# dscripka/openWakeWord

Hardware: AMD Instinct MI355X
Metric: real-time audio frames/sec (80 ms frame, 3 wakewords), whole job; real-time streams = value/12.5 (higher is better)
Workload: dtype f32 as 3xf16 split MFMA, fp32 accumulate; 1 GPU; 131072 concurrent 16 kHz streams per GPU x 3 heads (alexa,hey_mycroft,hey_jarvis), 80 ms frames, BASELINE configs[3] per-GPU shard; streams_per_gpu=131072, frame_samples=1280, collective=none, gather=none, rccl_ranks=0, pcm_distribution=Gaussian, RMS 3000, pcm=resident in HBM, kernels=mfma_rr_f16x3, graph=False, vad=off, weights=synthetic seed 1234, step_blocks=1

## Files before the change

### openwakeword_amd/csrc/owwhip.hip

```cpp
#include <hip/hip_runtime.h>

#include <algorithm>
#include <cmath>
#include <cstdio>
#include <cstdlib>
#include <cstring>
#include <ctime>
#include <exception>
#include <mutex>
#include <new>
#include <unordered_map>
#include <dlfcn.h>
#include <string>
#include <vector>

#include "owwhip.h"
#include "owwhip_pack.h"
#include "owwhip_kernels.h"
#include "owwhip_rr.h"
#include "owwhip_hx.h"
#include "owwhip_vad.h"
#include "owwhip_fused.h"
#include "owwhip_state.h"
#include "owwhip_events.h"
// ... 164 lines not shown
        oww_event* h_rec = nullptr; int* h_count = nullptr;
    };
    int evt_cap = 0, evt_rows = 0;
    float* d_evt_thr = nullptr; float evt_bank_thr = 0.5f;
    int* d_evblock = nullptr; int evt_blocks = 0;
    EventBuf evt_sync, evt_slot[2];
    const EventBuf* evt_cur = nullptr;

    hipStream_t up_stream = nullptr, down_stream = nullptr;
    uint64_t n_submit = 0, n_collect = 0;
    float* d_featinit = nullptr;
    float* d_dbg = nullptr;
    long long* d_prof = nullptr;
    int prof_block = -1;
    uint32_t *d_nfeat = nullptr, *d_npred = nullptr;
    float* d_vadring = nullptr; uint32_t* d_nvad = nullptr; float* d_vadin = nullptr; float vad_threshold = 0.f;
    bool vad = false;
    const float *d_vad_hann = nullptr, *d_vad_encw = nullptr, *d_vad_encb = nullptr, *d_vad_lstmw = nullptr, *d_vad_lstmb = nullptr, *d_vad_wd = nullptr;
    float vad_bd = 0.f, vad_gain = 50.f;
    float *d_vadx = nullptr, *d_vadhc = nullptr, *d_vadlast = nullptr;
    int16_t *d_tail = nullptr, *d_pcm = nullptr;
    int16_t* d_long = nullptr; size_t long_cap = 0;
    float* d_callmax = nullptr;
    int* h_range = nullptr;
    int* d_range = nullptr;
    void* d_rs = nullptr; size_t rs_bytes = 0;
    std::vector<float> rs_taps;
    uint8_t* d_on = nullptr;
    int* d_lists = nullptr; int* h_lists[2] = {nullptr, nullptr}; hipEvent_t lists_ev[2] = {nullptr, nullptr}; size_t lists_cap = 0; unsigned lists_turn = 0;
    int k_last = 1;
    float hx_absmax[20] = {};
    std::vector<int16_t> cal_user;
    int small_wgs = kSmallLaunchWgs, small_wgs_heads = kSmallLaunchWgs;
    float hx_selftest_err = 0.f, hx_selftest_ref = 0.f, hx_selftest_score_err = 0.f;
    bool fuse = false;
    float *d_verw = nullptr, *d_verb = nullptr, *d_verthr = nullptr; int* d_verT = nullptr;
    int ver_stride = 0, n_verifiers = 0;
    std::vector<int> ver_T;
    bool post_in_heads = false;
    float* d_save = nullptr; size_t save_floats = 0;
    int* d_ids = nullptr;
    int ids_cap = 0;
    int *d_patience = nullptr;
    float* d_threshold = nullptr;
    int debounce_frames = 0;
    void* comm = nullptr; int comm_rank = 0, comm_world = 1;
    bool timing = false;
    std::vector<EventRec> ev;
    size_t ev_used = 0;
    double t_ms[OWW_N_KERNEL_CLASSES] = {};
    int64_t t_n[OWW_N_KERNEL_CLASSES] = {};
    bool want_graph = false;
    hipGraph_t graph = nullptr;
    hipGraphExec_t graph_exec = nullptr;
    struct BankHead {
        bool live = false;
        int T = 0, hidden = 0, has_ln = 0, ht = 4, patience = 0;
        float threshold = NAN;
        float* d_img = nullptr;
        size_t w1_bytes = 0;
        owh::BankHeadDev dev{};
    };
    int bank_K = 0, bank_cap = 0;
    std::vector<BankHead> bank;
    std::vector<int> bank_sub;
    int* d_bank_sub = nullptr; int* d_bank_idx = nullptr;
// ... 102 lines not shown
            p.w[i] = h->d_conv[first_layer + i]; p.scale[i] = h->d_scale[first_layer + i];
            p.shift[i] = h->d_shift[first_layer + i]; p.dbg_off[i] = dbg_off[first_layer + i];
        }
        p.dbg = dbg ? h->d_dbg : nullptr; p.dbg_stride = DBG_FLOATS;
        p.prof = h->d_prof ? h->d_prof + (first_layer / 4) * 256 : nullptr;
        p.prof_block = h->prof_block;
    };
    {
        StageParams p{}; fill(p, h->d_xA, h->d_xB, 3, 2, 3);
        Timed t(h, 2);
        hipLaunchKernelGGL((stage_kernel<CfgB, MFMA, false>), dim3((n_active + CfgB::B - 1) / CfgB::B), dim3(CfgB::NT), CfgB::LDS_BYTES, st, p);
    }
    {
        StageParams p{}; fill(p, h->d_xB, h->d_xC, 7, 4, 5);
        Timed t(h, 3);
        hipLaunchKernelGGL((stage_kernel<CfgC, MFMA, false>), dim3((n_active + CfgC::B - 1) / CfgC::B), dim3(CfgC::NT), CfgC::LDS_BYTES, st, p);
    }
    {
        StageParams p{}; fill(p, h->d_xC, h->d_xD, 11, 6, 7);
        Timed t(h, 4);
        hipLaunchKernelGGL((stage_kernel<CfgD, MFMA, false>), dim3((n_active + CfgD::B - 1) / CfgD::B), dim3(CfgD::NT), CfgD::LDS_BYTES, st, p);
    }
    {
        StageParams p{}; fill(p, h->d_xD, nullptr, 15, 8, 9);
        p.hist19 = h->d_state[10]; p.w19 = h->d_conv[19]; p.feat = h->d_feat; p.emb = h->d_emb; p.nfeat = h->d_nfeat; p.TR = h->TR;
        p.dbg_off[4] = dbg_off[19];
        Timed t(h, 5);
        hipLaunchKernelGGL((stage_kernel<CfgE, MFMA, true>), dim3((n_active + CfgE::B - 1) / CfgE::B), dim3(CfgE::NT), CfgE::LDS_BYTES, st, p);
    }
    HIPCHK(hipGetLastError());
    return 0;
}

template <class CR, class CH, int WG, bool LAST, bool DBG, bool HX>
void launch_rstage(oww_ctx* h, const owr::RStageParams& p, int cls) {
    hipStream_t st = h->stream;
    Timed t(h, cls);
    const int nwg = (p.n_groups + WG - 1) / WG;
    if (HX && !DBG && nwg <= h->small_wgs) hipLaunchKernelGGL((owh::hstage_kernel<CH, LAST, false, WG, 3>), dim3(nwg), dim3(64 * WG), 0, st, p);
    else if (HX) hipLaunchKernelGGL((owh::hstage_kernel<CH, LAST, DBG, WG>), dim3(nwg), dim3(64 * WG), 0, st, p);
    else hipLaunchKernelGGL((owr::rstage_kernel<CR, LAST, DBG>), dim3((p.n_groups + 3) / 4), dim3(256), 0, st, p);
}

template <bool DBG, bool HX>
int run_cnn_rr(oww_ctx* h, const StepArgs& a, int n_active, int mel_stride, int mel_off) {
    using namespace owr;
    hipStream_t st = h->stream;
    int off = 0, dbg_off[20];
    for (int l = 0; l < 20; ++l) { dbg_off[l] = off; off += kLayerOut[l][0] * kLayerOut[l][1] * kLayerOut[l][2]; }
    {
        RAParams p{};
        p.mel = a.mel ? a.mel : h->d_mel; p.mel_stride = mel_stride; p.mel_off = mel_off;
        p.hist_mel = h->d_state[0]; p.hist2 = h->d_state[1];
        p.w0 = h->d_conv[0]; p.w1 = h->d_conv[1]; p.w2 = h->d_conv[2];
        for (int i = 0; i < 3; ++i) { p.scale[i] = h->d_scale[i]; p.shift[i] = h->d_shift[i]; p.dbg_off[i] = dbg_off[i]; }
        p.xout = h->d_xA; p.n_streams = n_active; p.S = h->Spad;
        p.dbg = DBG ? h->d_dbg : nullptr; p.dbg_stride = DBG_FLOATS;
        for (int i = 0; i < 3; ++i) { p.clampv[i] = -0.4f * ldexpf(1.f, h->hx_e[i]); p.dbg_mul[i] = ldexpf(1.f, -h->hx_e[i]); }
        p.xmul = ldexpf(1.f, h->hx_xexp[0]);
        p.range_flag = HX ? h->d_range : nullptr;
        p.stream_on = a.on;
        const int grid = std::min((n_active + 3) / 4, 768);
        Timed t(h, 1);
        if (HX && a.fused_pcm) {
            owf::MelAParams q{};
            q.a = p; q.a.mel = nullptr; q.a.n_streams = h->S;
            q.pcm = a.fused_pcm; q.tail = h->d_tail; q.nfeat = h->d_nfeat; q.hann = h->d_hann; q.mel_start = h->d_mstart; q.mel_taps = h->d_taps; q.mel_off = h->d_meloff; q.mel_dst = h->d_meldst;
            q.mel_out = h->cfg.debug_layers ? h->d_mel : nullptr;
            const int per_cu = std::max(1, std::min(12 / owf::FA_WG, 163840 / owf::FA_LDS_BYTES));
            const int g2 = std::max(1, std::min((q.a.n_streams + owf::FA_WG - 1) / owf::FA_WG, 256 * per_cu));
            hipLaunchKernelGGL(owf::hmelA_kernel<DBG>, dim3(g2), dim3(64 * owf::FA_WG), owf::FA_LDS_BYTES, st, q);
        }
        else if (HX) hipLaunchKernelGGL(owh::hstageA_kernel<DBG>, dim3(std::min((n_active + 3) / 4, 256 * OWH_WPS_A)), dim3(256), 0, st, p);
        else hipLaunchKernelGGL(rstageA_kernel<DBG>, dim3(grid), dim3(256), 0, st, p);
    }
    auto fill = [&](const float* xin, float* xout, int first_layer, int sb, int sd, int spt) {
        RStageParams p{};
        p.xin = xin; p.xout = xout; p.hist_b = h->d_state[sb]; p.hist_d = h->d_state[sd];
        for (int i = 0; i < 4; ++i) {
            p.w[i] = h->d_conv[first_layer + i]; p.scale[i] = h->d_scale[first_layer + i];
            p.shift[i] = h->d_shift[first_layer + i]; p.dbg_off[i] = dbg_off[first_layer + i];
            p.clampv[i] = -0.4f * ldexpf(1.f, h->hx_e[first_layer + i]); p.dbg_mul[i] = ldexpf(1.f, -h->hx_e[first_layer + i]);
        }
        p.dbg_mul[4] = ldexpf(1.f, -h->hx_e[19]);
        p.xmul = ldexpf(1.f, h->hx_xexp[first_layer / 4 + 1]);
        p.emb_mul = ldexpf(1.f, -h->hx_e[19]);
        p.n_groups = (n_active + spt - 1) / spt; p.S = h->Spad;
        p.dbg = DBG ? h->d_dbg : nullptr; p.dbg_stride = DBG_FLOATS;
        p.range_flag = HX ? h->d_range : nullptr;
        p.stream_on = a.on;
        if (HX && a.lists) {
            const int k = spt == 1 ? 0 : spt == 2 ? 1 : spt == 4 ? 2 : 3;
            p.glist = a.gl[k]; p.n_groups = a.gn[k];
        }
        return p;
    };
    launch_rstage<RB, owh::HB, OWH_WG_B, false, DBG, HX>(h, fill(h->d_xA, h->d_xB, 3, 2, 3, RB::SPT), 2);
    launch_rstage<RC, owh::HC, OWH_WG_C, false, DBG, HX>(h, fill(h->d_xB, h->d_xC, 7, 4, 5, RC::SPT), 3);
    launch_rstage<RD, owh::HD, OWH_WG_D, false, DBG, HX>(h, fill(h->d_xC, h->d_xD, 11, 6, 7, RD::SPT), 4);
    RStageParams pe = fill(h->d_xD, nullptr, 15, 8, 9, RE::SPT);
    pe.hist19 = h->d_state[10]; pe.w19 = h->d_conv[19]; pe.feat = h->d_feat; pe.emb = h->d_emb; pe.nfeat = h->d_nfeat; pe.TR = h->TR;
    pe.dbg_off[4] = dbg_off[19];
    launch_rstage<RE, owh::HE, OWH_WG_E, true, DBG, HX>(h, pe, 5);
    HIPCHK(hipGetLastError());
    return 0;
}

int run_cnn(oww_ctx* h, const StepArgs& a, int n_active, int mel_stride, int mel_off) {
    n_active = std::min(h->Spad, (n_active + 7) / 8 * 8);
    if (h->hx) return a.dbg ? run_cnn_rr<true, true>(h, a, n_active, mel_stride, mel_off) : run_cnn_rr<false, true>(h, a, n_active, mel_stride, mel_off);
    if (h->rr) return a.dbg ? run_cnn_rr<true, false>(h, a, n_active, mel_stride, mel_off) : run_cnn_rr<false, false>(h, a, n_active, mel_stride, mel_off);
    return h->mfma ? run_cnn_t<true>(h, a, n_active, mel_stride, mel_off) : run_cnn_t<false>(h, a, n_active, mel_stride, mel_off);
}

int heads_lds_bytes(int NH) { return (HD_SB * 100 + 2 * HD_SB * (NH + 4) + HD_SB * HD_MAXNETS) * 4; }

void launch_generic_heads(oww_ctx* h, const HeadParams& p, int n_active, int nb, int ne, hipStream_t st) {
    const int hs = (std::max(h->generic_hmax, 1) + 3) & ~3;
    const bool big = h->generic_hmax <= 128 && (h->generic_spw == 16 || (h->generic_spw == 0 && n_active >= GH_BIG_STREAMS));
    if (big) hipLaunchKernelGGL((heads_generic_kernel<16, 2, 2>), dim3((n_active + 31) / 32), dim3(128), gh_lds_bytes(16, 2, hs), st, p, nb, ne, hs);
    else hipLaunchKernelGGL((heads_generic_kernel<4, 4>), dim3((n_active + 15) / 16), dim3(256), gh_lds_bytes(4, 4, hs), st, p, nb, ne, hs);
}

int run_heads(oww_ctx* h, const StepArgs& a, int n_active, bool accumulate_max, const float* ext, int only_head, float* raw_out, int force_generic) {
    hipStream_t st = h->stream;
    Timed t(h, 6);
    HeadParams base{};
    base.feat = ext ? ext : h->d_feat; base.ext = ext ? 1 : 0; base.TR = h->TR; base.nfeat = h->d_nfeat;
    base.raw = raw_out; base.NL = h->NL; base.S = n_active; base.accumulate_max = accumulate_max ? 1 : 0;
    base.stream_on = ext ? nullptr : a.on;
    const bool fast_ok = h->mfma && !force_generic;
    if (fast_ok) {
        for (auto& g : h->groups) {
            if (only_head >= 0) {
                bool has = false;
                for (int ni : g.nets) has |= h->nets[ni].head == only_head;
// ... 881 lines not shown
        const size_t G = (SP + 15) / 16;
        if (int rc = dalloc(h->stream, &h->d_vadx, G * 4 * 1024)) return rc;
        if (int rc = dalloc(h->stream, &h->d_vadhc, G * 4096)) return rc;
        if (int rc = dalloc(h->stream, &h->d_vadlast, SP)) return rc;
    }
    if (int rc = dalloc(h->stream, &h->d_tail, SP * 480)) return rc;
    if (int rc = dalloc(h->stream, &h->d_pcm, (size_t)h->S * OWW_CHUNK * h->kmax)) return rc;
    if (int rc = dalloc(h->stream, &h->d_patience, (size_t)std::max(h->NL, 1))) return rc;
    if (int rc = dalloc(h->stream, &h->d_threshold, (size_t)std::max(h->NL, 1))) return rc;
    {
        std::vector<float> nanv(std::max(h->NL, 1), NAN);
        HIPCHK(copy_async(h->d_threshold, nanv.data(), nanv.size() * sizeof(float), hipMemcpyHostToDevice, h->stream));
    }
    if (h->cfg.debug_layers) if (int rc = dalloc(h->stream, &h->d_dbg, SP * DBG_FLOATS)) return rc;
    if (const char* e = getenv("OWW_PROF_BLOCK")) { h->prof_block = atoi(e); if (int rc = dalloc(h->stream, &h->d_prof, (size_t)4 * 256)) return rc; }
    return 0;
}

int set_kernel_lds(oww_ctx* h) {
    int rc = 0;
    auto lds = [&rc](auto kernel, int bytes) { if (!rc) rc = set_lds(kernel, bytes); };
    for (const auto& g : h->groups) if (g.ht == 4) lds(heads64_kernel, heads_lds_bytes(g.NH));
    if (!h->rnn_nets.empty()) lds(heads_rnn_kernel<RNN_SPW>, (int)rnn_lds_bytes(RNN_TMAX));
    if (h->vad) lds(owv::vad_front_kernel, owv::V_LDS_BYTES);
    lds(owf::hmelA_kernel<false>, owf::FA_LDS_BYTES); lds(owf::hmelA_kernel<true>, owf::FA_LDS_BYTES);
    lds(stageA_kernel<true>, CfgA::LDS_BYTES); lds(stageA_kernel<false>, CfgA::LDS_BYTES);
    lds(stage_kernel<CfgB, true, false>, CfgB::LDS_BYTES); lds(stage_kernel<CfgB, false, false>, CfgB::LDS_BYTES);
    lds(stage_kernel<CfgC, true, false>, CfgC::LDS_BYTES); lds(stage_kernel<CfgC, false, false>, CfgC::LDS_BYTES);
    lds(stage_kernel<CfgD, true, false>, CfgD::LDS_BYTES); lds(stage_kernel<CfgD, false, false>, CfgD::LDS_BYTES);
    lds(stage_kernel<CfgE, true, true>, CfgE::LDS_BYTES); lds(stage_kernel<CfgE, false, true>, CfgE::LDS_BYTES);
    return rc;
}

int derive_reset_state(oww_ctx* h, const HxCalib& cal, CommitClock& clk) {
    const size_t SP = h->Spad;
    const int warm = std::min<int>(32, (int)SP);
    hipLaunchKernelGGL(fill_kernel, dim3((warm * 256 + 255) / 256), dim3(256), 0, h->stream, h->d_mel, (size_t)warm * 256, 1.0f);
    const StepArgs args{};
    for (int it = 0; it < 12; ++it)
        if (int rc = run_cnn(h, args, warm, 256, 0)) return rc;
    for (int a = 0; a < N_STATE; ++a)
        HIPCHK(copy_async(h->d_tmpl[a], h->d_state[a], (size_t)h->state_len[a] * (h->rr ? kStateSpgRr[a] : 1) * sizeof(float),
                              hipMemcpyDeviceToDevice, h->stream));
    HIPCHK(hipMemsetAsync(h->d_mel, 0, SP * 8 * h->kmax * 32 * sizeof(float), h->stream));
    HIPCHK(hipMemsetAsync(h->d_emb, 0, SP * 96 * sizeof(float), h->stream));
    if (int rc = do_reset(h, nullptr, (int)SP, nullptr)) return rc;
    HIPCHK(hipStreamSynchronize(h->stream));
    clk.lap("warm-up + reset");
    if (int rc = range_check(h, "oww_commit")) return rc;
    if (h->hx && !getenv("OWW_NO_COMMIT_SELFTEST")) {
        if (int rc = selftest_hx(h, cal)) return rc;
        HIPCHK(hipMemsetAsync(h->d_mel, 0, SP * 8 * h->kmax * 32 * sizeof(float), h->stream));
        HIPCHK(hipMemsetAsync(h->d_emb, 0, SP * 96 * sizeof(float), h->stream));
        HIPCHK(hipMemsetAsync(h->d_raw, 0, SP * std::max(h->NL, 1) * sizeof(float), h->stream));
        if (int rc = do_reset(h, nullptr, (int)SP, nullptr)) return rc;
        HIPCHK(hipStreamSynchronize(h->stream));
        clk.lap("self-test replay + reset");
    }
    return 0;
}

int alloc_bank(oww_ctx* h) {
    const size_t SK = (size_t)h->S * h->bank_K;
    if (int rc = dalloc(h->stream, &h->d_bank_sub, SK, false)) return rc;
    if (int rc = dalloc(h->stream, &h->d_bank_idx, SK)) return rc;
    if (int rc = dalloc(h->stream, &h->d_bank_raw, SK)) return rc;
// ... 330 lines not shown
    if (int rc = build_nets(*h, h->NL, h->TR, h->generic_hmax)) return rc;
    if (h->evt_rows > h->TR)
        return fail(OWW_EINVAL, "oww_events_configure: feature_rows = %d exceeds the handle's feature ring (%d rows)", h->evt_rows, h->TR);
    CommitClock clk(h->hx ? "f16-split" : "family");
    HxCalib cal;
    if (h->hx) {
        if (int rc = calibrate_hx(h, cal)) return rc;
        h->probe_emb = cal.ref_emb; h->probe_nb = cal.nb;
        clk.lap("calibration (total)");
        if (getenv("OWW_DEBUG_CALIB"))
            for (int l = 0; l < 20; ++l) fprintf(stderr, "calib layer %2d: max|a| %-12.5g e_in %4d e_out %4d\n", l, h->hx_absmax[l], h->hx_ein[l], h->hx_e[l]);
    }
    HostBuf hb;
    WeightOff off;
    HeadGroups hg;
    h->no_wide_heads = getenv("OWW_NO_WIDE_HEADS") != nullptr;
    if (int rc = pack_mel_tables(*h, hb, off)) return rc;
    if (int rc = pack_cnn(*h, hb, off)) return rc;
    pack_net_arrays(*h, hb, off);
    if (int rc = pack_head_groups(*h, hg, hb, off)) return rc;
    h->groups.clear();
    for (const HeadGroup& g : hg.groups) h->groups.push_back(FastGroup{g});
    h->generic_nets = hg.generic_nets; h->rnn_nets = hg.rnn_nets;
    h->vad = !h->vad_blob.empty();
    if (int rc = pack_vad(*h, hb, off, h->vad_gain, h->vad_bd)) return rc;
    clk.lap("weight packing (host)");
    if (int rc = bind_weights(h, hb, off)) return rc;
    if (int rc = alloc_range_flag(h)) return rc;
    clk.lap("weight upload");
    if (int rc = alloc_state(h)) return rc;
    h->fuse = h->hx && !getenv("OWW_NO_FUSE");
    if (const char* e = getenv("OWW_SMALL_WGS")) h->small_wgs = atoi(e);
    if (const char* e = getenv("OWW_SMALL_WGS_HEADS")) h->small_wgs_heads = atoi(e);
    if (const char* e = getenv("OWW_GENERIC_SPW")) { const int v = atoi(e); h->generic_spw = v == 4 || v == 16 ? v : 0; }
    h->post_in_heads = h->fuse && h->groups.size() == 1 && h->groups[0].ht == 4 && h->generic_nets.empty() && h->rnn_nets.empty() && h->NL > 0;
    if (int rc = set_kernel_lds(h)) return rc;
    clk.lap("state allocation");
    if (int rc = derive_reset_state(h, cal, clk)) return rc;
    if (h->bank_K > 0) if (int rc = alloc_bank(h)) return rc;
    if (h->vpool_cap > 0) if (int rc = alloc_verifiers(h)) return rc;
    if (events_on(h)) if (int rc = alloc_events(h)) return rc;
    h->committed = true;
    return OWW_OK;
    OWW_GUARD_END
}

int oww_reset(oww_ctx* h, const int32_t* stream_ids, int32_t n, const float* init_features) {
    OWW_GUARD_BEGIN
    if (!h || !h->committed) return fail(OWW_ESTATE, "oww_reset: handle not committed");
    HIPCHK(hipSetDevice(h->cfg.device));
    const float* d_init = nullptr;
    if (init_features) {
        HIPCHK(copy_async(h->d_featinit, init_features, (size_t)h->TR * 96 * sizeof(float), hipMemcpyHostToDevice, h->stream));
        d_init = h->d_featinit;
    }
    if (!stream_ids) {
        if (int rc = do_reset(h, nullptr, h->Spad, d_init)) return rc;
    } else {
        if (n < 1) return OWW_OK;
        for (int i = 0; i < n; ++i)
            if (stream_ids[i] < 0 || stream_ids[i] >= h->S) return fail(OWW_EINVAL, "oww_reset: stream id %d out of range", stream_ids[i]);
        if (n > h->ids_cap) {
            if (h->d_ids) (void)dev_free(h->d_ids);
            h->d_ids = nullptr; h->ids_cap = 0;
            HIPCHK(dev_alloc(&h->d_ids, (size_t)n * sizeof(int)));
            h->ids_cap = n;
// ... 1284 lines not shown
```

### openwakeword_amd/csrc/owwhip_hx.h

```cpp
#pragma once
#include <type_traits>
#include <utility>
#include "owwhip_layout.h"
#include "owwhip_rr.h"

namespace owh {

using owr::f32x4;
typedef _Float16 f16x8 __attribute__((ext_vector_type(8)));

constexpr float WUNSCALE = 1.0f / 256.0f;

__device__ __forceinline__ float act1(float x, float cl) {
    return fmaxf(fmaxf(0.2f * x, x), cl);
}
template <bool ACT, bool HALF>
__device__ __forceinline__ f32x4 act_t(const f32x4 v, float cl) {
    if (!ACT) return HALF ? f32x4{v[0], v[1], 0.f, 0.f} : v;
    if (HALF) return f32x4{act1(v[0], cl), act1(v[1], cl), 0.f, 0.f};
    return f32x4{act1(v[0], cl), act1(v[1], cl), act1(v[2], cl), act1(v[3], cl)};
}
template <bool HALF>
__device__ __forceinline__ void pin_t(f32x4& v) {
    if (!HALF) { owr::pin(v); return; }
// ... 671 lines not shown
            }
#pragma unroll
            for (int r = 0; r < NR; ++r) {
                if (HOUT && oct == NCTO) { out[r][oct - 1] = act_t<BN, true>(prev[r], cl); pin_t<true>(out[r][oct - 1]); }
                else { out[r][oct - 1] = act_t<BN, false>(prev[r], cl); pin_t<false>(out[r][oct - 1]); }
            }
        }
#if OWH_PIPE_M
        if (oct > 0 && oct < NCTO) {
#pragma unroll
            for (int i = 0; i < 3 * (3 * KSF + NMK) * NR; ++i) {
                __builtin_amdgcn_sched_group_barrier(0x008, 1, 0);
                __builtin_amdgcn_sched_group_barrier(0x002, OWH_PIPE_VALU, 0);
            }
        }
#endif
        if (oct < NCTO) {
#pragma unroll
            for (int r = 0; r < NR; ++r) prev[r] = acc[r];
                ring_end<NS, NBLK, NCTO, NEXT_NBLK, WG>(oct);
        }
    }
}

#ifndef OWH_HIST_LDS
#define OWH_HIST_LDS 1
#endif
#ifndef OWH_HIST_LDS_C
#define OWH_HIST_LDS_C 0
#endif
#ifndef OWH_SPRIO_B
#define OWH_SPRIO_B 1111
#endif
#ifndef OWH_SPRIO_C
#define OWH_SPRIO_C 3210
#endif
#ifndef OWH_SPRIO_D
#define OWH_SPRIO_D 3210
#endif
#ifndef OWH_SPRIO_E
#define OWH_SPRIO_E 1111
#endif
template <int CODE, int LAYER> __device__ __forceinline__ void sprio() {
    constexpr int div = LAYER == 0 ? 1000 : LAYER == 1 ? 100 : LAYER == 2 ? 10 : 1;
    if constexpr (CODE != 0 && LAYER >= 0) __builtin_amdgcn_s_setprio((CODE / div) % 10);
    if constexpr (CODE != 0 && LAYER < 0) __builtin_amdgcn_s_setprio(0);
}
template <int NBLK>
__device__ __forceinline__ void issue_hist(const float* __restrict__ gsrc, float* ldst, int lane) {
    const float* base = owr::uniform_ptr(gsrc);
#pragma unroll
    for (int i = 0; i < NBLK; ++i)
        __builtin_amdgcn_global_load_lds((const __attribute__((address_space(1))) void*)(base + i * 256 + lane * 4),
                                         (__attribute__((address_space(3))) void*)(ldst + i * 256), 16, 0, 0);
}
template <int NCT, bool HALF>
__device__ __forceinline__ void load_tile_lds(f32x4 (&t)[NCT], const float* base, int lane) {
#pragma unroll
    for (int ct = 0; ct < NCT; ++ct)
#pragma unroll
        for (int e = 0; e < 4; ++e) {
            if (HALF && ct == NCT - 1 && e >= 2) t[ct][e] = 0.f;
            else t[ct][e] = base[(ct * 4 + e) * 64 + lane];
        }
}

template <class C, bool LAST, bool DBG, int WG = OWH_WG, int NS = 2>
__global__ __launch_bounds__(64 * WG, (DBG || NS > 3 ? 1 : (NS == 3 && C::WPS > 2 ? 2 : C::WPS))) void hstage_kernel(owr::RStageParams p) {
    using namespace owr;
    constexpr int NCTI = C::NCTI, NCT = C::NCT, R = C::RP, F = C::F;
    static_assert(!LAST || C::NPASS == 1, "the last stage runs in one pass");
    static_assert(NS == 2 || C::NPASS == 1 || (4 * NCT) % NS == 0, "multi-pass stages need a ring phase that returns to 0 after each pass");
    static_assert(NS >= 2 && NS <= 5 && NS - 1 <= NCT, "the chunks in flight at a layer boundary belong to at most the next layer");
    constexpr int KSA = (NCTI + 1) / 2, KS = (NCT + 1) / 2;
    constexpr int NBA = 3 * KSA * 2, NB = 3 * KS * 2;
    using TK = TimeK<NCT, C::HOUT>;
    constexpr bool MERGE = OWH_KMERGE && (NCT % 2 == 1) && !LAST && (C::HOUT || OWH_KMERGE_B);
    constexpr int NBT = MERGE ? TK::NBLK : NB;
    constexpr bool PIPE = OWH_PIPE != 0;
    constexpr int APCFG = NCT == 3 ? OWH_APIPE_B : NCT == 5 ? OWH_APIPE_C : LAST ? OWH_APIPE_E : OWH_APIPE_D;
    constexpr bool APM = (APCFG & 1) != 0, APT = (APCFG & 2) != 0;
    constexpr int SPCODE = NCT == 3 ? OWH_SPRIO_B : NCT == 5 ? OWH_SPRIO_C : LAST ? OWH_SPRIO_E : OWH_SPRIO_D;
    constexpr bool REM2 = OWH_REM2 && NCT % 2 == 1 && !C::HOUT && !LAST && !(OWH_KMERGE && OWH_KMERGE_B) && !(OWH_KMERGE_MEL && OWH_KMERGE_MEL2B);
    constexpr bool MMA2 = OWH_KMERGE_MEL && OWH_KMERGE_MEL2 && kInterleave && !C::HIN && NCTI % 2 == 1 && NCTI >= 3 && C::WPS == 2;
    constexpr bool MMA = (OWH_KMERGE_MEL && kInterleave && C::HIN && NCTI % 2 == 1 && NCTI >= 3) || MMA2;
    constexpr int NPRA = MMA2 ? 2 : 1, NMKA = (3 * NPRA + 3) / 4;
    constexpr bool MMC2 = OWH_KMERGE_MEL && OWH_KMERGE_MEL2B && !C::HOUT && NCT % 2 == 1 && NCT >= 3 && !LAST;
    constexpr bool MMC = (OWH_KMERGE_MEL && kInterleave && C::HOUT && NCT % 2 == 1 && NCT >= 3) || MMC2;
    constexpr int NPRC = MMC2 ? 2 : 1, NMKC = (3 * NPRC + 3) / 4;
    constexpr int NBAM = MMA ? (3 * (KSA - 1) + NMKA) * 2 : NBA, NBCM = MMC ? (3 * (KS - 1) + NMKC) * 2 : NB;
    constexpr int NBMAX = (NBAM > NBT ? NBAM : NBT) > (NBCM > (LAST ? NB : 0) ? NBCM : (LAST ? NB : 0)) ? (NBAM > NBT ? NBAM : NBT) : (NBCM > (LAST ? NB : 0) ? NBCM : (LAST ? NB : 0));
    constexpr int WBS = NBMAX * 256;
    constexpr bool HLDS = OWH_HIST_LDS && !LAST && C::NPASS == 1 && (C::SPT == 1 || (C::SPT == 2 && OWH_HIST_LDS_C));
    constexpr int HROW = NCT * 4 * 64;
    const int lane = threadIdx.x & 63;
    const int wave = __builtin_amdgcn_readfirstlane(threadIdx.x >> 6);
    int g = blockIdx.x * WG + wave;
    __shared__ __attribute__((aligned(16))) float wbuf[WBS];
    __shared__ __attribute__((aligned(16))) float wbuf1[WBS];
    __shared__ __attribute__((aligned(16))) float wbuf2[NS >= 3 ? WBS : 4];
    __shared__ __attribute__((aligned(16))) float wbuf3[NS >= 4 ? WBS : 4];
    __shared__ __attribute__((aligned(16))) float wbuf4[NS >= 5 ? WBS : 4];
    const WRing<NS> ring{{wbuf, wbuf1, wbuf2, wbuf3, wbuf4}};
    __shared__ __attribute__((aligned(16))) float sbn[4][NCT * 16];
    __shared__ __attribute__((aligned(16))) float hlds[HLDS ? WG * 2 * HROW : 4];
    float* const hl = hlds + (HLDS ? wave * 2 * HROW : 0);
    const bool active = g < p.n_groups;
    if (!active) g = p.n_groups - 1;
    if (p.glist) g = p.glist[g];
    else g += p.g_base;
    lanemask_t bad = 0;
    ring_issue<NS, NBAM, WG>(p.w[0], wbuf, wave, lane);
    if (NS >= 3) ring_issue<NS, NBAM, WG>(p.w[0] + (size_t)NBAM * 256, wbuf1, wave, lane);
    if (NS >= 4) ring_issue<NS, NBAM, WG>(p.w[0] + (size_t)2 * NBAM * 256, wbuf2, wave, lane);
    if (NS >= 5) ring_issue<NS, NBAM, WG>(p.w[0] + (size_t)3 * NBAM * 256, wbuf3, wave, lane);
    for (int i = threadIdx.x; i < 4 * NCT * 16; i += 64 * WG) {
        const int l = i / (NCT * 16), c = i % (NCT * 16);
        sbn[l][c] = p.shift[l][c];
    }
    const int s_first = g * C::SPT;
    const bool lane_on = active && (p.stream_on == nullptr || p.stream_on[min(s_first + tile_stream<F>(lane & 15), p.S - 1)] != 0);
    float* hb = p.hist_b + (size_t)g * C::HIST_FLOATS;
    float* hd = p.hist_d + (size_t)g * C::HIST_FLOATS;
    if (HLDS) issue_hist<2 * NCT>(hb, hl, lane);

#pragma unroll
    for (int pass = 0; pass < C::NPASS; ++pass) {
    f32x4 Y[R][NCT];
    Op Xo[R][KSA];
#pragma unroll
    for (int r = 0; r < R; ++r) {
        f32x4 X[NCTI];
        load_tile_h<NCTI, C::HIN>(X, p.xin + ((size_t)price_alias<(OWH_PRICE_HANDOVER & 2) != 0 && C::CIN == 24>(g) * C::R + pass * R + r) * (NCTI * 4 * 64), lane);
        to_ops<NCTI, C::HIN>(X, Xo[r]);
    }
    if (pass == 0) chunk_sync();
    sprio<SPCODE, 0>();

    if constexpr (MMA) {
        Op Mx[R][NMKA];
        merge_mel_rems<KSA, R, F, NPRA>(Xo, Mx);
        conv_mel_hxm<KSA, NMKA, NCT, R, F, true, 0, NBT, WG, C::HOUT, NS, APM>(Xo, Mx, Y, ring, p.w[0], p.w[1], sbn[0], p.clampv[0], wave, lane, bad);
    } else
    conv_mel_hx<KSA, NCT, R, F, true, 0, NBT, WG, C::HOUT, false, NS, APM>(Xo, Y, ring, p.w[0], p.w[1], sbn[0], p.clampv[0], wave, lane, bad);
    if (DBG && p.dbg && active) {
#pragma unroll
        for (int r = 0; r < R; ++r) dump_tile_ht<NCT, F, C::C>(Y[r], p.dbg, p.dbg_stride, p.dbg_off[0], s_first, pass * R + r, p.S, lane, p.dbg_mul[0]);
    }
    Op Ao[R][KS], H0[KS], H1[KS];
    sprio<SPCODE, 1>();
    if constexpr (MERGE) {
        Op AoF[R][TK::KSF], H0F[TK::KSF], H1F[TK::KSF], M[R][TK::NMK];
        RemPairs rem[R + 2];
        {
            f32x4 T0[NCT], T1[NCT];
            if (HLDS) { load_tile_lds<NCT, C::HOUT>(T0, hl, lane); load_tile_lds<NCT, C::HOUT>(T1, hl + HROW, lane); }
            else { load_tile_h<NCT, C::HOUT>(T0, hb, lane); load_tile_h<NCT, C::HOUT>(T1, hb + NCT * 4 * 64, lane); }
            to_ops_time<NCT, C::HOUT>(T0, H0F, rem[0]);
            to_ops_time<NCT, C::HOUT>(T1, H1F, rem[1]);
        }
        if (HLDS) { asm volatile("s_waitcnt lgkmcnt(0)" ::: "memory"); issue_hist<2 * NCT>(hd, hl, lane); }
        if (lane_on) {
            store_tile_h<NCT, C::HOUT>(Y[R - 2], hb, lane);
            store_tile_h<NCT, C::HOUT>(Y[R - 1], hb + NCT * 4 * 64, lane);
        }
#pragma unroll
        for (int r = 0; r < R; ++r) to_ops_time<NCT, C::HOUT>(Y[r], AoF[r], rem[2 + r]);
        merge_rems<R, TK::NPR, TK::NMK>(rem, M);
        __builtin_amdgcn_sched_barrier(0);
// ... 15 lines not shown
    for (int r = 0; r < R; ++r) to_ops<NCT, C::HOUT, REM2>(Y[r], Ao[r]);
    __builtin_amdgcn_sched_barrier(0);
    conv_time_hx<KS, NCT, R, true, NCT, NBCM, WG, true, C::HOUT, PIPE, REM2, NS, APT>(H0, H1, Ao, Y, ring, p.w[1], p.w[2], sbn[1], p.clampv[1], wave, lane, bad);
    }
    if (DBG && p.dbg && active) {
#pragma unroll
        for (int r = 0; r < R; ++r) dump_tile_ht<NCT, F, C::C>(Y[r], p.dbg, p.dbg_stride, p.dbg_off[1], s_first, pass * R + r, p.S, lane, p.dbg_mul[1]);
    }
#pragma unroll
    for (int r = 0; r < R; ++r) to_ops<NCT, C::HOUT, REM2>(Y[r], Ao[r]);
    __builtin_amdgcn_sched_barrier(0);
    sprio<SPCODE, 2>();
    if constexpr (MMC) {
        Op Mc[R][NMKC];
        merge_mel_rems<KS, R, F, NPRC>(Ao, Mc);
        conv_mel_hxm<KS, NMKC, NCT, R, F, true, 2 * NCT, NBT, WG, C::HOUT, NS, APM>(Ao, Mc, Y, ring, p.w[2], p.w[3], sbn[2], p.clampv[2], wave, lane, bad);
    } else
    conv_mel_hx<KS, NCT, R, F, true, 2 * NCT, NBT, WG, C::HOUT, REM2, NS, APM>(Ao, Y, ring, p.w[2], p.w[3], sbn[2], p.clampv[2], wave, lane, bad);
    if (DBG && p.dbg && active) {
#pragma unroll
        for (int r = 0; r < R; ++r) dump_tile_ht<NCT, F, C::C>(Y[r], p.dbg, p.dbg_stride, p.dbg_off[2], s_first, pass * R + r, p.S, lane, p.dbg_mul[2]);
    }
    sprio<SPCODE, 3>();
    if constexpr (MERGE) {
        Op AoF[R][TK::KSF], H0F[TK::KSF], H1F[TK::KSF], M[R][TK::NMK];
        RemPairs rem[R + 2];
        {
            f32x4 T0[NCT], T1[NCT];
            if (HLDS) { load_tile_lds<NCT, C::HOUT>(T0, hl, lane); load_tile_lds<NCT, C::HOUT>(T1, hl + HROW, lane); }
            else { load_tile_h<NCT, C::HOUT>(T0, hd, lane); load_tile_h<NCT, C::HOUT>(T1, hd + NCT * 4 * 64, lane); }
            to_ops_time<NCT, C::HOUT>(T0, H0F, rem[0]);
            to_ops_time<NCT, C::HOUT>(T1, H1F, rem[1]);
        }
        if (lane_on) {
            store_tile_h<NCT, C::HOUT>(Y[R - 2], hd, lane);
            store_tile_h<NCT, C::HOUT>(Y[R - 1], hd + NCT * 4 * 64, lane);
        }
#pragma unroll
        for (int r = 0; r < R; ++r) to_ops_time<NCT, C::HOUT>(Y[r], AoF[r], rem[2 + r]);
        merge_rems<R, TK::NPR, TK::NMK>(rem, M);
        __builtin_amdgcn_sched_barrier(0);
        conv_time_hxm<TK::KSF, TK::NMK, NCT, R, true, 3 * NCT, (C::NPASS > 1 ? NBAM : 0), WG, C::HOUT, NS, APT>(H0F, H1F, AoF, M, Y, ring, p.w[3], p.w[0], sbn[3], p.clampv[3], wave, lane, bad);
    } else {
    {
        f32x4 T0[NCT], T1[NCT];
        if (HLDS) { load_tile_lds<NCT, C::HOUT>(T0, hl, lane); load_tile_lds<NCT, C::HOUT>(T1, hl + HROW, lane); }
        else { load_tile_h<NCT, C::HOUT>(T0, hd, lane); load_tile_h<NCT, C::HOUT>(T1, hd + NCT * 4 * 64, lane); }
        to_ops<NCT, C::HOUT, REM2>(T0, H0);
        to_ops<NCT, C::HOUT, REM2>(T1, H1);
    }
    if (lane_on) {
        store_tile_h<NCT, C::HOUT>(Y[R - 2], hd, lane);
        store_tile_h<NCT, C::HOUT>(Y[R - 1], hd + NCT * 4 * 64, lane);
    }
#pragma unroll
    for (int r = 0; r < R; ++r) to_ops<NCT, C::HOUT, REM2>(Y[r], Ao[r]);
    __builtin_amdgcn_sched_barrier(0);
    conv_time_hx<KS, NCT, R, true, 3 * NCT, (LAST ? NB : (C::NPASS > 1 ? NBAM : 0)), WG, true, C::HOUT, PIPE, REM2, NS, APT>(H0, H1, Ao, Y, ring, p.w[3], LAST ? p.w19 : p.w[0], sbn[3], p.clampv[3], wave, lane, bad);
    }
    if (DBG && p.dbg && active) {
#pragma unroll
        for (int r = 0; r < R; ++r) dump_tile_ht<NCT, F, C::C>(Y[r], p.dbg, p.dbg_stride, p.dbg_off[3], s_first, pass * R + r, p.S, lane, p.dbg_mul[3]);
    }

    sprio<SPCODE, -1>();
    if (!LAST && lane_on) {
        constexpr int FO = C::FO, RO = C::RO;
        constexpr int SPTN = 16 / FO;
        const int pos = lane & 15, j = lane >> 4;
        const int sp = tile_stream<F>(pos), f = tile_mel<F>(pos);
        const int s = g * C::SPT + sp;
        const int gn = s / SPTN, spn = s % SPTN;
        const int posn = tile_pos<FO>(spn, f / 2);
        constexpr int SH = kInterleave ? C::SPT : 1;
#pragma unroll
        for (int ro = 0; ro < R / C::PT; ++ro) {
            float pm[NCT][4];
#pragma unroll
            for (int ct = 0; ct < NCT; ++ct)
#pragma unroll
                for (int e = 0; e < 4; ++e) {
                    if (C::HOUT && ct == NCT - 1 && e >= 2) { pm[ct][e] = 0.f; continue; }
                    float m = Y[ro * C::PT][ct][e];
                    if (C::PT == 2) m = fmax_nc(m, Y[ro * C::PT + 1][ct][e]);
                    pm[ct][e] = fmax_nc(m, dpp_shl_zero<SH>(m)) * p.xmul;
                }
            if ((f & 1) == 0) {
                float* xo = p.xout + ((size_t)(gn * RO + pass * (R / C::PT) + ro) * (NCT * 4)) * 64 + j * 16 + posn;
#pragma unroll
                for (int ct = 0; ct < NCT; ++ct)
#pragma unroll
                    for (int e = 0; e < 4; ++e)
                        if (!(C::HOUT && ct == NCT - 1 && e >= 2)) xo[(ct * 4 + e) * 64] = pm[ct][e];
            }
        }
    }
    if (LAST) {
        static_assert(!LAST || (C::RO == 1 && C::FO == 1 && NCT == 6), "last stage pools to one position, 96 channels");
        const int pos = lane & 15, j = lane >> 4;
        f32x4 Pl[NCT];
        const int src = (j * 16 + tile_pos<F>(pos & 7, 0)) * 4;
        constexpr int SH = kInterleave ? C::SPT : 1;
#pragma unroll
        for (int ct = 0; ct < NCT; ++ct)
#pragma unroll
            for (int e = 0; e < 4; ++e) {
                float m = fmax_nc(Y[0][ct][e], Y[1][ct][e]);
                m = fmax_nc(m, dpp_shl_zero<SH>(m)) * p.xmul;
                Pl[ct][e] = __builtin_bit_cast(float, __builtin_amdgcn_ds_bpermute(src, __builtin_bit_cast(int, m)));
            }
        float* h19 = p.hist19 + (size_t)g * (2 * NCT * 4 * 64);
        f32x4 T0[NCT], T1[NCT];
        Op H0[KS], H1[KS];
        load_tile<NCT>(T0, h19, lane);
        load_tile<NCT>(T1, h19 + NCT * 4 * 64, lane);
        to_ops<NCT>(T0, H0);
        to_ops<NCT>(T1, H1);
        Op Po[1][KS];
        to_ops<NCT>(Pl, Po[0]);
        f32x4 E[1][NCT];
        conv_time_hx<KS, NCT, 1, false, 4 * NCT, 0, WG, false, false, OWH_PIPE != 0, false, NS>(H0, H1, Po, E, ring, p.w19, nullptr, nullptr, 0.f, wave, lane, bad);
        const bool on19 = active && (p.stream_on == nullptr || p.stream_on[min(s_first + (pos & 7), p.S - 1)] != 0);
        if (on19) {
            store_tile<NCT>(T1, h19, lane);
            store_tile<NCT>(Pl, h19 + NCT * 4 * 64, lane);
        }
        const int s = s_first + pos;
        if (on19 && pos < C::SPT && s < p.S) {
            const uint32_t slot = p.nfeat[s] % (uint32_t)p.TR;
#pragma unroll
            for (int ct = 0; ct < NCT; ++ct) {
                const f32x4 ev = E[0][ct] * p.emb_mul;
                *reinterpret_cast<f32x4*>(p.feat + ((size_t)s * p.TR + slot) * 96 + ct * 16 + 4 * j) = ev;
                *reinterpret_cast<f32x4*>(p.emb + (size_t)s * 96 + ct * 16 + 4 * j) = ev;
                if (DBG && p.dbg) *reinterpret_cast<f32x4*>(p.dbg + (size_t)s * p.dbg_stride + p.dbg_off[4] + ct * 16 + 4 * j) = ev;
            }
        }
    }
    }
    if (!LAST && C::NPASS > 1) asm volatile("s_waitcnt vmcnt(0)" ::: "memory");
    raise_range_flag(bad, p.range_flag, s_first, C::SPT);
}

#ifndef OWF_QPRIO
#if !defined(OWF_PRIO) || OWF_PRIO == 6
#define OWF_QPRIO 2233
#else
#define OWF_QPRIO 0
#endif
#endif
namespace sa {
constexpr int RS = 34;
constexpr int PLANE = 344;
constexpr int WAVE_HALVES = 2 * PLANE;
}
typedef unsigned u32x4 __attribute__((ext_vector_type(4)));

__device__ __forceinline__ void stageA_fill_gather_table(int* gtab , int tid, int nt) {
    for (int i = tid; i < 512; i += nt) {
        const int lane = i >> 3, q = i & 7, p = lane & 15, g = lane >> 4, slot = 8 * g + q;
        const int tap = slot % 9, plane = slot >= 18 ? 1 : 0;
        gtab[i] = slot < 27 ? 2 * (plane * sa::PLANE + (tap / 3) * sa::RS + (tap % 3) + 2 * p) : 0;
    }
}
__device__ __forceinline__ void stageA_put_mel(_Float16* sP, int row, int bin, float v) {
    const _Float16 hi = (_Float16)v;
    sP[row * sa::RS + 1 + bin] = hi;
    sP[sa::PLANE + row * sa::RS + 1 + bin] = (_Float16)(v - (float)hi);
}
__device__ __forceinline__ f32x4 mfma3(const f16x8 ah, const f16x8 al, const Op& x, f32x4 c) {
    c = OWH_MFMA(ah, x.h, c);
    c = OWH_MFMA(ah, x.l, c);
    return OWH_MFMA(al, x.h, c);
}
// ... 1132 lines not shown
```

Before: 24.04 million frames/s.

## Add persistent grid-stride form of CNN stage kernels C and D

Adds a persistent variant of the hstage kernel. The grid is sized from an occupancy query (blocks per CU times CU count) and each workgroup loops over several stream groups. Across units it keeps the weight ring prefetch chained, issues the next group's history load into LDS early, and skips the initial chunk sync after the first unit. The intent is to amortize the per-block prologue (weight prefetch, shift table load, launch overhead) and overlap history loads with compute. It is on by default for stages C and D. The cost is more register and control complexity, and possible load imbalance with a fixed grid.

```diff
diff --git a/openwakeword_amd/csrc/owwhip.hip b/openwakeword_amd/csrc/owwhip.hip
--- a/openwakeword_amd/csrc/owwhip.hip
+++ b/openwakeword_amd/csrc/owwhip.hip
@@ -220,6 +220,8 @@
     float hx_absmax[20] = {};
     std::vector<int16_t> cal_user;
     int small_wgs = kSmallLaunchWgs, small_wgs_heads = kSmallLaunchWgs;
+    int persist_wgs[4] = {0, 0, 0, 0};
+    int stage_persist = 15, stage_grid = 0;
     float hx_selftest_err = 0.f, hx_selftest_ref = 0.f, hx_selftest_score_err = 0.f;
     bool fuse = false;
     float *d_verw = nullptr, *d_verb = nullptr, *d_verthr = nullptr; int* d_verT = nullptr;
@@ -388,12 +390,17 @@
     return 0;
 }
 
-template <class CR, class CH, int WG, bool LAST, bool DBG, bool HX>
+template <class CR, class CH, int WG, bool LAST, bool DBG, bool HX, bool PERSIST>
 void launch_rstage(oww_ctx* h, const owr::RStageParams& p, int cls) {
     hipStream_t st = h->stream;
     Timed t(h, cls);
     const int nwg = (p.n_groups + WG - 1) / WG;
+    int pgrid = PERSIST && HX && !DBG && ((h->stage_persist >> (cls - 2)) & 1) ? h->persist_wgs[cls - 2] : 0;
+    if (pgrid > 0 && h->stage_grid > 0) pgrid = std::min(pgrid, h->stage_grid);
     if (HX && !DBG && nwg <= h->small_wgs) hipLaunchKernelGGL((owh::hstage_kernel<CH, LAST, false, WG, 3>), dim3(nwg), dim3(64 * WG), 0, st, p);
+    else if (PERSIST && HX && !DBG && pgrid > 0) {
+        if constexpr (PERSIST && HX && !DBG) hipLaunchKernelGGL((owh::hstage_kernel<CH, LAST, false, WG, 2, true>), dim3(std::min(nwg, pgrid)), dim3(64 * WG), 0, st, p);
+    }
     else if (HX) hipLaunchKernelGGL((owh::hstage_kernel<CH, LAST, DBG, WG>), dim3(nwg), dim3(64 * WG), 0, st, p);
     else hipLaunchKernelGGL((owr::rstage_kernel<CR, LAST, DBG>), dim3((p.n_groups + 3) / 4), dim3(256), 0, st, p);
 }
@@ -451,13 +458,13 @@
         }
         return p;
     };
-    launch_rstage<RB, owh::HB, OWH_WG_B, false, DBG, HX>(h, fill(h->d_xA, h->d_xB, 3, 2, 3, RB::SPT), 2);
-    launch_rstage<RC, owh::HC, OWH_WG_C, false, DBG, HX>(h, fill(h->d_xB, h->d_xC, 7, 4, 5, RC::SPT), 3);
-    launch_rstage<RD, owh::HD, OWH_WG_D, false, DBG, HX>(h, fill(h->d_xC, h->d_xD, 11, 6, 7, RD::SPT), 4);
+    launch_rstage<RB, owh::HB, OWH_WG_B, false, DBG, HX, OWH_PERSIST_B != 0>(h, fill(h->d_xA, h->d_xB, 3, 2, 3, RB::SPT), 2);
+    launch_rstage<RC, owh::HC, OWH_WG_C, false, DBG, HX, OWH_PERSIST_C != 0>(h, fill(h->d_xB, h->d_xC, 7, 4, 5, RC::SPT), 3);
+    launch_rstage<RD, owh::HD, OWH_WG_D, false, DBG, HX, OWH_PERSIST_D != 0>(h, fill(h->d_xC, h->d_xD, 11, 6, 7, RD::SPT), 4);
     RStageParams pe = fill(h->d_xD, nullptr, 15, 8, 9, RE::SPT);
     pe.hist19 = h->d_state[10]; pe.w19 = h->d_conv[19]; pe.feat = h->d_feat; pe.emb = h->d_emb; pe.nfeat = h->d_nfeat; pe.TR = h->TR;
     pe.dbg_off[4] = dbg_off[19];
-    launch_rstage<RE, owh::HE, OWH_WG_E, true, DBG, HX>(h, pe, 5);
+    launch_rstage<RE, owh::HE, OWH_WG_E, true, DBG, HX, OWH_PERSIST_E != 0>(h, pe, 5);
     HIPCHK(hipGetLastError());
     return 0;
 }
@@ -1405,6 +1412,24 @@
     return rc;
 }
 
+int query_stage_residency(oww_ctx* h) {
+    hipDeviceProp_t prop;
+    HIPCHK(hipGetDeviceProperties(&prop, h->cfg.device));
+    int rc = 0;
+    auto q = [&](int i, auto kernel, int wg) {
+        int per_cu = 0;
+        if (rc) return;
+        if (hipOccupancyMaxActiveBlocksPerMultiprocessor(&per_cu, kernel, 64 * wg, 0) != hipSuccess) rc = fail(OWW_EHIP, "persistent stage kernels: occupancy query failed");
+        else h->persist_wgs[i] = std::max(1, per_cu) * prop.multiProcessorCount;
+    };
+    if constexpr (OWH_PERSIST_B != 0) q(0, owh::hstage_kernel<owh::HB, false, false, OWH_WG_B, 2, true>, OWH_WG_B);
+    if constexpr (OWH_PERSIST_C != 0) q(1, owh::hstage_kernel<owh::HC, false, false, OWH_WG_C, 2, true>, OWH_WG_C);
+    if constexpr (OWH_PERSIST_D != 0) q(2, owh::hstage_kernel<owh::HD, false, false, OWH_WG_D, 2, true>, OWH_WG_D);
+    if constexpr (OWH_PERSIST_E != 0) q(3, owh::hstage_kernel<owh::HE, true, false, OWH_WG_E, 2, true>, OWH_WG_E);
+    if (getenv("OWW_DEBUG_PERSIST")) fprintf(stderr, "persistent stage grids B..E: %d %d %d %d\n", h->persist_wgs[0], h->persist_wgs[1], h->persist_wgs[2], h->persist_wgs[3]);
+    return rc;
+}
+
 int derive_reset_state(oww_ctx* h, const HxCalib& cal, CommitClock& clk) {
     const size_t SP = h->Spad;
     const int warm = std::min<int>(32, (int)SP);
@@ -1801,6 +1826,9 @@
     h->fuse = h->hx && !getenv("OWW_NO_FUSE");
     if (const char* e = getenv("OWW_SMALL_WGS")) h->small_wgs = atoi(e);
     if (const char* e = getenv("OWW_SMALL_WGS_HEADS")) h->small_wgs_heads = atoi(e);
+    if (const char* e = getenv("OWW_STAGE_PERSIST")) h->stage_persist = atoi(e);
+    if (const char* e = getenv("OWW_STAGE_GRID")) h->stage_grid = std::max(0, atoi(e));
+    if (h->hx) if (int rc = query_stage_residency(h)) return rc;
     if (const char* e = getenv("OWW_GENERIC_SPW")) { const int v = atoi(e); h->generic_spw = v == 4 || v == 16 ? v : 0; }
     h->post_in_heads = h->fuse && h->groups.size() == 1 && h->groups[0].ht == 4 && h->generic_nets.empty() && h->rnn_nets.empty() && h->NL > 0;
     if (int rc = set_kernel_lds(h)) return rc;
diff --git a/openwakeword_amd/csrc/owwhip_hx.h b/openwakeword_amd/csrc/owwhip_hx.h
--- a/openwakeword_amd/csrc/owwhip_hx.h
+++ b/openwakeword_amd/csrc/owwhip_hx.h
@@ -727,6 +727,9 @@
 #ifndef OWH_SPRIO_B
 #define OWH_SPRIO_B 1111
 #endif
+#ifndef OWH_SPRIO_B_PERSIST
+#define OWH_SPRIO_B_PERSIST 3210
+#endif
 #ifndef OWH_SPRIO_C
 #define OWH_SPRIO_C 3210
 #endif
@@ -760,11 +763,34 @@
         }
 }
 
-template <class C, bool LAST, bool DBG, int WG = OWH_WG, int NS = 2>
-__global__ __launch_bounds__(64 * WG, (DBG || NS > 3 ? 1 : (NS == 3 && C::WPS > 2 ? 2 : C::WPS))) void hstage_kernel(owr::RStageParams p) {
+#ifndef OWH_PERSIST_B
+#define OWH_PERSIST_B 0
+#endif
+#ifndef OWH_PERSIST_C
+#define OWH_PERSIST_C 1
+#endif
+#ifndef OWH_PERSIST_D
+#define OWH_PERSIST_D 1
+#endif
+#ifndef OWH_PERSIST_E
+#define OWH_PERSIST_E 0
+#endif
+#ifndef OWH_PERSIST_HIST_EARLY
+#define OWH_PERSIST_HIST_EARLY 1
+#endif
+typedef const __attribute__((address_space(4))) owr::RStageParams KernargStageParams;
+template <bool K, class A, class B> __device__ __forceinline__ decltype(auto) pick_ref(A& a, B& b) {
+    if constexpr (K) return (a); else return (b);
+}
+template <class C, bool LAST, bool DBG, int WG = OWH_WG, int NS = 2, bool PERSIST = false>
+__global__ __launch_bounds__(64 * WG, (DBG || NS > 3 ? 1 : (NS == 3 && C::WPS > 2 ? 2 : C::WPS))) void hstage_kernel(owr::RStageParams pk) {
     using namespace owr;
+    KernargStageParams* kp = (KernargStageParams*)__builtin_amdgcn_kernarg_segment_ptr();
+    const owr::RStageParams& p = pk;
     constexpr int NCTI = C::NCTI, NCT = C::NCT, R = C::RP, F = C::F;
     static_assert(!LAST || C::NPASS == 1, "the last stage runs in one pass");
+    static_assert(!PERSIST || (NS == 2 && !DBG), "the persistent form is the two-slot production kernel");
+    static_assert(!PERSIST || ((4 * NCT * C::NPASS + (LAST ? NCT : 0)) % NS == 0), "the ring phase returns to slot 0 after each unit");
     static_assert(NS == 2 || C::NPASS == 1 || (4 * NCT) % NS == 0, "multi-pass stages need a ring phase that returns to 0 after each pass");
     static_assert(NS >= 2 && NS <= 5 && NS - 1 <= NCT, "the chunks in flight at a layer boundary belong to at most the next layer");
     constexpr int KSA = (NCTI + 1) / 2, KS = (NCT + 1) / 2;
@@ -775,7 +801,7 @@
     constexpr bool PIPE = OWH_PIPE != 0;
     constexpr int APCFG = NCT == 3 ? OWH_APIPE_B : NCT == 5 ? OWH_APIPE_C : LAST ? OWH_APIPE_E : OWH_APIPE_D;
     constexpr bool APM = (APCFG & 1) != 0, APT = (APCFG & 2) != 0;
-    constexpr int SPCODE = NCT == 3 ? OWH_SPRIO_B : NCT == 5 ? OWH_SPRIO_C : LAST ? OWH_SPRIO_E : OWH_SPRIO_D;
+    constexpr int SPCODE = NCT == 3 ? (PERSIST ? OWH_SPRIO_B_PERSIST : OWH_SPRIO_B) : NCT == 5 ? OWH_SPRIO_C : LAST ? OWH_SPRIO_E : OWH_SPRIO_D;
     constexpr bool REM2 = OWH_REM2 && NCT % 2 == 1 && !C::HOUT && !LAST && !(OWH_KMERGE && OWH_KMERGE_B) && !(OWH_KMERGE_MEL && OWH_KMERGE_MEL2B);
     constexpr bool MMA2 = OWH_KMERGE_MEL && OWH_KMERGE_MEL2 && kInterleave && !C::HIN && NCTI % 2 == 1 && NCTI >= 3 && C::WPS == 2;
     constexpr bool MMA = (OWH_KMERGE_MEL && kInterleave && C::HIN && NCTI % 2 == 1 && NCTI >= 3) || MMA2;
@@ -788,9 +814,8 @@
     constexpr int WBS = NBMAX * 256;
     constexpr bool HLDS = OWH_HIST_LDS && !LAST && C::NPASS == 1 && (C::SPT == 1 || (C::SPT == 2 && OWH_HIST_LDS_C));
     constexpr int HROW = NCT * 4 * 64;
-    const int lane = threadIdx.x & 63;
-    const int wave = __builtin_amdgcn_readfirstlane(threadIdx.x >> 6);
-    int g = blockIdx.x * WG + wave;
+    const int lane0 = threadIdx.x & 63, lane = lane0;
+    const int wave0 = __builtin_amdgcn_readfirstlane(threadIdx.x >> 6), wave = wave0;
     __shared__ __attribute__((aligned(16))) float wbuf[WBS];
     __shared__ __attribute__((aligned(16))) float wbuf1[WBS];
     __shared__ __attribute__((aligned(16))) float wbuf2[NS >= 3 ? WBS : 4];
@@ -799,12 +824,11 @@
     const WRing<NS> ring{{wbuf, wbuf1, wbuf2, wbuf3, wbuf4}};
     __shared__ __attribute__((aligned(16))) float sbn[4][NCT * 16];
     __shared__ __attribute__((aligned(16))) float hlds[HLDS ? WG * 2 * HROW : 4];
-    float* const hl = hlds + (HLDS ? wave * 2 * HROW : 0);
-    const bool active = g < p.n_groups;
-    if (!active) g = p.n_groups - 1;
-    if (p.glist) g = p.glist[g];
-    else g += p.g_base;
-    lanemask_t bad = 0;
+    auto unit_group = [&](const auto& p, int u) {
+        const int gi = min(u * WG + wave, p.n_groups - 1);
+        if (p.glist) return p.glist[gi];
+        return gi + p.g_base;
+    };
     ring_issue<NS, NBAM, WG>(p.w[0], wbuf, wave, lane);
     if (NS >= 3) ring_issue<NS, NBAM, WG>(p.w[0] + (size_t)NBAM * 256, wbuf1, wave, lane);
     if (NS >= 4) ring_issue<NS, NBAM, WG>(p.w[0] + (size_t)2 * NBAM * 256, wbuf2, wave, lane);
@@ -813,11 +837,25 @@
         const int l = i / (NCT * 16), c = i % (NCT * 16);
         sbn[l][c] = p.shift[l][c];
     }
+    int unit = blockIdx.x;
+    do {
+    int lane_u = lane0, wave_u = wave0;
+    if (PERSIST) asm volatile("" : "+s"(kp), "+v"(lane_u), "+s"(wave_u));
+    const int wave = PERSIST ? min(wave_u, WG - 1) : wave0;
+    float* const hl = hlds + (HLDS ? wave * 2 * HROW : 0);
+    const int lane = lane_u & 63;
+    const auto& p = pick_ref<PERSIST>(*kp, pk);
+    const bool first_unit = !PERSIST || unit == (int)blockIdx.x;
+    lanemask_t bad = 0;
+    const bool active = unit * WG + wave < p.n_groups;
+    const int g = unit_group(p, unit);
     const int s_first = g * C::SPT;
     const bool lane_on = active && (p.stream_on == nullptr || p.stream_on[min(s_first + tile_stream<F>(lane & 15), p.S - 1)] != 0);
     float* hb = p.hist_b + (size_t)g * C::HIST_FLOATS;
     float* hd = p.hist_d + (size_t)g * C::HIST_FLOATS;
-    if (HLDS) issue_hist<2 * NCT>(hb, hl, lane);
+    if (HLDS && (first_unit || !OWH_PERSIST_HIST_EARLY)) issue_hist<2 * NCT>(hb, hl, lane);
+    const float* hb_next = hb;
+    if (PERSIST && HLDS) hb_next = p.hist_b + (size_t)unit_group(p, (unit + (int)gridDim.x) * WG < p.n_groups ? unit + (int)gridDim.x : unit) * C::HIST_FLOATS;
 
 #pragma unroll
     for (int pass = 0; pass < C::NPASS; ++pass) {
@@ -829,7 +867,7 @@
         load_tile_h<NCTI, C::HIN>(X, p.xin + ((size_t)price_alias<(OWH_PRICE_HANDOVER & 2) != 0 && C::CIN == 24>(g) * C::R + pass * R + r) * (NCTI * 4 * 64), lane);
         to_ops<NCTI, C::HIN>(X, Xo[r]);
     }
-    if (pass == 0) chunk_sync();
+    if (pass == 0 && first_unit) chunk_sync();
     sprio<SPCODE, 0>();
 
     if constexpr (MMA) {
@@ -911,6 +949,7 @@
             to_ops_time<NCT, C::HOUT>(T0, H0F, rem[0]);
             to_ops_time<NCT, C::HOUT>(T1, H1F, rem[1]);
         }
+        if (PERSIST && HLDS && OWH_PERSIST_HIST_EARLY) { asm volatile("s_waitcnt lgkmcnt(0)" ::: "memory"); issue_hist<2 * NCT>(hb_next, hl, lane); }
         if (lane_on) {
             store_tile_h<NCT, C::HOUT>(Y[R - 2], hd, lane);
             store_tile_h<NCT, C::HOUT>(Y[R - 1], hd + NCT * 4 * 64, lane);
@@ -919,7 +958,7 @@
         for (int r = 0; r < R; ++r) to_ops_time<NCT, C::HOUT>(Y[r], AoF[r], rem[2 + r]);
         merge_rems<R, TK::NPR, TK::NMK>(rem, M);
         __builtin_amdgcn_sched_barrier(0);
-        conv_time_hxm<TK::KSF, TK::NMK, NCT, R, true, 3 * NCT, (C::NPASS > 1 ? NBAM : 0), WG, C::HOUT, NS, APT>(H0F, H1F, AoF, M, Y, ring, p.w[3], p.w[0], sbn[3], p.clampv[3], wave, lane, bad);
+        conv_time_hxm<TK::KSF, TK::NMK, NCT, R, true, 3 * NCT, (C::NPASS > 1 || PERSIST ? NBAM : 0), WG, C::HOUT, NS, APT>(H0F, H1F, AoF, M, Y, ring, p.w[3], p.w[0], sbn[3], p.clampv[3], wave, lane, bad);
     } else {
     {
         f32x4 T0[NCT], T1[NCT];
@@ -928,6 +967,7 @@
         to_ops<NCT, C::HOUT, REM2>(T0, H0);
         to_ops<NCT, C::HOUT, REM2>(T1, H1);
     }
+    if (PERSIST && HLDS && OWH_PERSIST_HIST_EARLY) { asm volatile("s_waitcnt lgkmcnt(0)" ::: "memory"); issue_hist<2 * NCT>(hb_next, hl, lane); }
     if (lane_on) {
         store_tile_h<NCT, C::HOUT>(Y[R - 2], hd, lane);
         store_tile_h<NCT, C::HOUT>(Y[R - 1], hd + NCT * 4 * 64, lane);
@@ -935,7 +975,7 @@
 #pragma unroll
     for (int r = 0; r < R; ++r) to_ops<NCT, C::HOUT, REM2>(Y[r], Ao[r]);
     __builtin_amdgcn_sched_barrier(0);
-    conv_time_hx<KS, NCT, R, true, 3 * NCT, (LAST ? NB : (C::NPASS > 1 ? NBAM : 0)), WG, true, C::HOUT, PIPE, REM2, NS, APT>(H0, H1, Ao, Y, ring, p.w[3], LAST ? p.w19 : p.w[0], sbn[3], p.clampv[3], wave, lane, bad);
+    conv_time_hx<KS, NCT, R, true, 3 * NCT, (LAST ? NB : (C::NPASS > 1 || PERSIST ? NBAM : 0)), WG, true, C::HOUT, PIPE, REM2, NS, APT>(H0, H1, Ao, Y, ring, p.w[3], LAST ? p.w19 : p.w[0], sbn[3], p.clampv[3], wave, lane, bad);
     }
     if (DBG && p.dbg && active) {
 #pragma unroll
@@ -998,7 +1038,7 @@
         Op Po[1][KS];
         to_ops<NCT>(Pl, Po[0]);
         f32x4 E[1][NCT];
-        conv_time_hx<KS, NCT, 1, false, 4 * NCT, 0, WG, false, false, OWH_PIPE != 0, false, NS>(H0, H1, Po, E, ring, p.w19, nullptr, nullptr, 0.f, wave, lane, bad);
+        conv_time_hx<KS, NCT, 1, false, 4 * NCT, (PERSIST ? NBAM : 0), WG, false, false, OWH_PIPE != 0, false, NS>(H0, H1, Po, E, ring, p.w19, PERSIST ? p.w[0] : nullptr, nullptr, 0.f, wave, lane, bad);
         const bool on19 = active && (p.stream_on == nullptr || p.stream_on[min(s_first + (pos & 7), p.S - 1)] != 0);
         if (on19) {
             store_tile<NCT>(T1, h19, lane);
@@ -1017,8 +1057,11 @@
         }
     }
     }
-    if (!LAST && C::NPASS > 1) asm volatile("s_waitcnt vmcnt(0)" ::: "memory");
+    if (!LAST && C::NPASS > 1 && !PERSIST) asm volatile("s_waitcnt vmcnt(0)" ::: "memory");
     raise_range_flag(bad, p.range_flag, s_first, C::SPT);
+    if (PERSIST && (unit += (int)gridDim.x) * WG >= p.n_groups) break;
+    } while (PERSIST);
+    if (PERSIST) asm volatile("s_waitcnt vmcnt(0)" ::: "memory");
 }
 
 #ifndef OWF_QPRIO
```

Result: no change. 24.19 million frames/s, median of 6 (+0.6%).
